# LogicTronixInc/Event-Camera-Clustering-and-Optical-Flow-Estimation

Measured on AMD Instinct MI355X. Metric: Mevents/s (downsample+cluster+corner), higher is better.
Workload: dtype u16xy/i64t (int), fp32 k-means; 1 GPU; e2e hash-downsample(8192-event windows) -> k-means k=16 (10 iters) on reps -> SAE+FAST arc corners (16384-event slices) -> 15x15 NMS; 346x260 sensor; 20004864 events/GPU/step (BASELINE configs C2-C4); events_per_gpu=20004864, events_total=20004864, preset=c4, reps_per_gpu=7697279, width=346, height=260, k=16, kmeans_iters=10, parallelism=time-window shards x1, launch=eager launches, streams=two streams sharing all CUs

## Files before the change

### event-camera-clustering-and-optical-flow-estimation_amd/csrc/corner_flags.hip

```cpp
#include "corner_common.hpp"
#include "flag_decode.hpp"

namespace {

#ifndef ECC_FLAG_THREADS
#define ECC_FLAG_THREADS 256
#endif
constexpr int kFlagThreads = ECC_FLAG_THREADS;
#ifndef ECC_FLAG_QUADS
#define ECC_FLAG_QUADS 8
#endif
constexpr int kFlagQuads = ECC_FLAG_QUADS;
constexpr int kFlagBatch = kFlagQuads * kFlagThreads;

#ifndef ECC_FLAG_GROUP
#define ECC_FLAG_GROUP 4
#endif
constexpr int kFlagGroup = ECC_FLAG_GROUP;
static_assert(kFlagQuads % kFlagGroup == 0, "a batch is whole read groups");
static_assert(kFlagTile == (uint32_t)kTile && kFlagSegWords == (uint32_t)kSegWords, "flag_decode.hpp's tile");

template <bool kStaged>
__device__ __forceinline__ uint32_t seg_word(uint32_t w, const uint32_t *sb, const uint32_t *__restrict__ rg) {
    return kStaged ? sb[w] : rg[w];
}

template <bool kStaged>
__device__ __forceinline__ uint32_t corner_bit(uint32_t v, const CornerGeom &g, uint32_t last_word, const uint32_t *sb,
                                               const uint32_t *__restrict__ rg) {
    const uint32_t x = (uint32_t)ecc::xy_x(v), y = (uint32_t)ecc::xy_y(v);
    const FlagSlot sl = flag_slot(x, y, (uint32_t)g.tiles_x, last_word);
    return (seg_word<kStaged>(sl.word, sb, rg) >> sl.bit) & flag_on_sensor(x, y, (uint32_t)g.W, (uint32_t)g.H);
}

__device__ __forceinline__ uint32_t first_bytes(int r) {
    const int rc = min(max(r, 0), 4);
    return rc >= 4 ? 0x01010101u : (0x01010101u & ((1u << (8 * (rc & 3))) - 1u));
}

template <bool kStaged, bool kCand>
__global__ void __launch_bounds__(kFlagThreads)
flags_event_kernel(const uint32_t *__restrict__ xy, CornerGeom g, const uint32_t *__restrict__ res,
                   const int32_t *__restrict__ first_border, uint8_t *__restrict__ flags, uint32_t *__restrict__ cand,
                   int32_t *__restrict__ n_cand) {
    extern __shared__ uint32_t sb[];
    __shared__ int ctot[kFlagQuads][kFlagThreads / 64];
    const int64_t s = blockIdx.x;
    const int64_t lo = s * g.S;
    const int len = (int)((lo + g.S < g.n ? lo + g.S : g.n) - lo);
    const uint32_t last_word = (uint32_t)(g.n_tiles * kSegWords - 1);
    const int live_end = s < g.first_detect ? 0 : (g.border_mode == 1 ? min(len, max(first_border[s], 0)) : len);
    const uint32_t *rg = res + s * g.seg_stride;
    const bool vec = ((lo + (int64_t)(reinterpret_cast<uintptr_t>(flags) & 3)) & 3) == 0;
    const int n4 = vec ? len / 4 : 0;
    const int lane = threadIdx.x & 63, wave = threadIdx.x >> 6;
    const __amdgpu_buffer_rsrc_t vq = ecc::buffer_view(xy + lo, (uint32_t)n4 * 16u);
    uint4 pre[kFlagQuads];
    auto load_batch = [&](int q0) {
#pragma unroll
        for (int u = 0; u < kFlagQuads; ++u)
            pre[u] = ecc::buffer_load_u128(vq, threadIdx.x * 16u, (uint32_t)(q0 + u * kFlagThreads) * 16u);
        __builtin_amdgcn_sched_barrier(0);
    };
    load_batch(0);
    if (kStaged && live_end > 0) {
        const int total = g.n_tiles * kSegWords;
        const __amdgpu_buffer_rsrc_t vr = ecc::buffer_view(rg, (uint32_t)total * 4u);
        for (int k0 = 0; k0 < total; k0 += 16 * kFlagThreads) {
            uint4 a[4];
#pragma unroll
            for (int b = 0; b < 4; ++b) a[b] = ecc::buffer_load_u128(vr, (uint32_t)(k0 + 4 * (b * kFlagThreads + (int)threadIdx.x)) * 4u);
            __builtin_amdgcn_sched_barrier(0);
#pragma unroll
            for (int b = 0; b < 4; ++b) {
                const int k = k0 + 4 * (b * kFlagThreads + (int)threadIdx.x);
                if (k + 3 < total) {
                    *reinterpret_cast<uint4 *>(sb + k) = a[b];
                } else {
                    if (k < total) sb[k] = a[b].x;
                    if (k + 1 < total) sb[k + 1] = a[b].y;
                    if (k + 2 < total) sb[k + 2] = a[b].z;
                }
            }
        }
    }
    __syncthreads();
    const int live_q = min(live_end, 4 * n4);
    const __amdgpu_buffer_rsrc_t vf = ecc::buffer_view(flags + lo, (uint32_t)n4 * 4u);
    const uint64_t lt = lane == 0 ? 0ull : (~0ull >> (64 - lane));
    int base = 0;
    uint32_t *dst = cand + lo;
    for (int q0 = 0; q0 < n4; q0 += kFlagBatch) {
        if (q0 > 0) load_batch(q0);
        uint32_t f[kFlagQuads];
        int pfx[kFlagQuads];
#pragma unroll
        for (int u0 = 0; u0 < kFlagQuads; u0 += kFlagGroup) {
            uint32_t wd[kFlagGroup][4], sh[kFlagGroup], ok[kFlagGroup];
#pragma unroll
            for (int u = 0; u < kFlagGroup; ++u) {
                const uint32_t ev[4] = {pre[u0 + u].x, pre[u0 + u].y, pre[u0 + u].z, pre[u0 + u].w};
                sh[u] = ok[u] = 0u;
#pragma unroll
                for (int k = 0; k < 4; ++k) {
                    const uint32_t x = (uint32_t)ecc::xy_x(ev[k]), y = (uint32_t)ecc::xy_y(ev[k]);
                    const FlagSlot sl = flag_slot(x, y, (uint32_t)g.tiles_x, last_word);
                    wd[u][k] = seg_word<kStaged>(sl.word, sb, rg);
                    sh[u] |= sl.bit << (8 * k);
                    ok[u] |= flag_on_sensor(x, y, (uint32_t)g.W, (uint32_t)g.H) << (8 * k);
                }
            }
#pragma unroll
            for (int u = 0; u < kFlagGroup; ++u) {
                const int i = 4 * (q0 + (u0 + u) * kFlagThreads + (int)threadIdx.x);
                uint32_t bits = 0u;
#pragma unroll
                for (int k = 0; k < 4; ++k) bits |= ((wd[u][k] >> ((sh[u] >> (8 * k)) & 31u)) & 1u) << (8 * k);
                f[u0 + u] = bits & ok[u] & first_bytes(live_q - i);
                ecc::buffer_store_u32(f[u0 + u], vf, threadIdx.x * 4u, (uint32_t)(q0 + (u0 + u) * kFlagThreads) * 4u);
            }
        }
#pragma unroll
        for (int u = 0; u < kFlagQuads; ++u) {
            if constexpr (kCand) {
                const int c = __popc(f[u]);
                const uint64_t b0 = __ballot(c & 1), b1 = __ballot(c & 2), b2 = __ballot(c & 4);
                pfx[u] = __popcll(b0 & lt) + 2 * __popcll(b1 & lt) + 4 * __popcll(b2 & lt);
                if (lane == 0) ctot[u][wave] = __popcll(b0) + 2 * __popcll(b1) + 4 * __popcll(b2);
            }
        }
        if constexpr (kCand) {
            __syncthreads();
#pragma unroll
            for (int u = 0; u < kFlagQuads; ++u) {
                int off = base + pfx[u];
#pragma unroll
                for (int w = 0; w < kFlagThreads / 64; ++w) {
                    const int tw = ctot[u][w];
                    off += w < wave ? tw : 0;
                    base += tw;
                }
                if (f[u]) {
                    if (f[u] & 0x1u) dst[off++] = pre[u].x;
                    if (f[u] & 0x100u) dst[off++] = pre[u].y;
                    if (f[u] & 0x10000u) dst[off++] = pre[u].z;
                    if (f[u] & 0x1000000u) dst[off++] = pre[u].w;
                }
            }
            __syncthreads();
        }
    }
    if constexpr (kCand) {
        if (threadIdx.x == 0) {
            for (int i = 4 * n4; i < len; ++i) {
                const uint32_t v = xy[lo + i];
                const uint32_t fb = corner_bit<kStaged>(v, g, last_word, sb, rg) & (i < live_end ? 1u : 0u);
                flags[lo + i] = (uint8_t)fb;
                if (fb) dst[base++] = v;
            }
            n_cand[s] = base;
        }
    } else {
        for (int i = 4 * n4 + threadIdx.x; i < len; i += kFlagThreads)
            flags[lo + i] = (uint8_t)(corner_bit<kStaged>(xy[lo + i], g, last_word, sb, rg) & (i < live_end ? 1u : 0u));
    }
}

}

int ecc::corner::launch_flags(ecc_ctx *ctx, hipStream_t s, const uint32_t *xy, const CornerGeom &g, const GroupImages &gi,
                              const int32_t *first_border, uint8_t *corner_flags, uint32_t *cand, int32_t *n_cand) {
    ECC_TIMED(ctx, s, "flags_kernel");
    constexpr size_t kLdsMax = kFlagDynLdsMax;
    const size_t lds = (size_t)g.n_tiles * kSegWords * sizeof(uint32_t);
    if (lds <= kLdsMax) {
        const auto fn = cand ? &flags_event_kernel<true, true> : &flags_event_kernel<true, false>;
        if (lds > 65536)
            if (int rc = ecc::allow_dynamic_lds(ctx, fn, (int)kLdsMax, "flags LDS")) return rc;
        if (cand)
            hipLaunchKernelGGL((flags_event_kernel<true, true>), dim3((unsigned)g.n_slices), dim3(kFlagThreads), lds, s,
                               xy, g, (const uint32_t *)gi.res, first_border, corner_flags, cand, n_cand);
        else
            hipLaunchKernelGGL((flags_event_kernel<true, false>), dim3((unsigned)g.n_slices), dim3(kFlagThreads), lds,
                               s, xy, g, (const uint32_t *)gi.res, first_border, corner_flags, nullptr, nullptr);
    } else {
        if (cand) return ECC_ERR_INVALID;
        hipLaunchKernelGGL((flags_event_kernel<false, false>), dim3((unsigned)g.n_slices), dim3(kFlagThreads), 0, s,
                           xy, g, (const uint32_t *)gi.res, first_border, corner_flags, nullptr, nullptr);
    }
    return ECC_OK;
}
```

Measured before the change: 44250 Mevents/s.

## Re-raster staged corner flags into sensor-order LDS bitmap, pipeline loads, pack scan

```diff
diff --git a/event-camera-clustering-and-optical-flow-estimation_amd/csrc/corner_flags.hip b/event-camera-clustering-and-optical-flow-estimation_amd/csrc/corner_flags.hip
--- a/event-camera-clustering-and-optical-flow-estimation_amd/csrc/corner_flags.hip
+++ b/event-camera-clustering-and-optical-flow-estimation_amd/csrc/corner_flags.hip
@@ -1,5 +1,6 @@
 #include "corner_common.hpp"
 #include "flag_decode.hpp"
+#include "flag_raster.hpp"
 
 namespace {
 
@@ -11,13 +12,36 @@
 #define ECC_FLAG_QUADS 8
 #endif
 constexpr int kFlagQuads = ECC_FLAG_QUADS;
-constexpr int kFlagBatch = kFlagQuads * kFlagThreads;
 
 #ifndef ECC_FLAG_GROUP
 #define ECC_FLAG_GROUP 4
 #endif
 constexpr int kFlagGroup = ECC_FLAG_GROUP;
 static_assert(kFlagQuads % kFlagGroup == 0, "a batch is whole read groups");
+#ifndef ECC_FLAG_RASTER
+#define ECC_FLAG_RASTER 1
+#endif
+constexpr bool kFlagRaster = ECC_FLAG_RASTER != 0;
+#ifndef ECC_FLAG_SCAN
+#define ECC_FLAG_SCAN 1
+#endif
+constexpr bool kFlagScan = ECC_FLAG_SCAN != 0;
+#ifndef ECC_FLAG_PIPE
+#define ECC_FLAG_PIPE 1
+#endif
+constexpr bool kFlagPipe = ECC_FLAG_PIPE != 0;
+static_assert(kFlagQuads % 2 == 0, "the quad counts are packed in pairs");
+constexpr int kFlagWaves = kFlagThreads / 64;
+constexpr int kFlagTotWords = kFlagScan ? 2 * kFlagWaves * (kFlagQuads / 2) : kFlagQuads * kFlagWaves;
+static_assert(kFlagTotWords * 4 + 4 <= 160 * 1024 - (int)kFlagDynLdsMax, "the static LDS kFlagDynLdsMax leaves room for");
+
+constexpr uint32_t kFlagListExtra = 384;
+__host__ __device__ inline uint32_t flag_lds_words(uint32_t n_tiles) {
+    const uint32_t seg = n_tiles * (uint32_t)kSegWords;
+    if (!kFlagRaster) return seg;
+    const uint32_t most = (uint32_t)(kFlagDynLdsMax / 4), want = ((seg + 3u) & ~3u) + kFlagListExtra;
+    return want < most ? want : most;
+}
 static_assert(kFlagTile == (uint32_t)kTile && kFlagSegWords == (uint32_t)kSegWords, "flag_decode.hpp's tile");
 
 template <bool kStaged>
@@ -25,12 +49,35 @@
     return kStaged ? sb[w] : rg[w];
 }
 
+template <bool kRaster>
+__device__ __forceinline__ FlagSlot flag_look(uint32_t x, uint32_t y, const CornerGeom &g, uint32_t last) {
+    if constexpr (kRaster) {
+        const uint32_t idx = flag_raster_index(x, y, (uint32_t)g.W, last);
+        return FlagSlot{idx >> 5, idx & 31u};
+    } else {
+        return flag_slot(x, y, (uint32_t)g.tiles_x, last);
+    }
+}
+
 template <bool kStaged>
-__device__ __forceinline__ uint32_t corner_bit(uint32_t v, const CornerGeom &g, uint32_t last_word, const uint32_t *sb,
+__device__ __forceinline__ uint32_t corner_bit(uint32_t v, const CornerGeom &g, uint32_t last, const uint32_t *sb,
                                                const uint32_t *__restrict__ rg) {
     const uint32_t x = (uint32_t)ecc::xy_x(v), y = (uint32_t)ecc::xy_y(v);
-    const FlagSlot sl = flag_slot(x, y, (uint32_t)g.tiles_x, last_word);
+    const FlagSlot sl = flag_look<kStaged && kFlagRaster>(x, y, g, last);
     return (seg_word<kStaged>(sl.word, sb, rg) >> sl.bit) & flag_on_sensor(x, y, (uint32_t)g.W, (uint32_t)g.H);
+}
+
+__device__ __forceinline__ void raster_or_word(uint32_t *sb, uint32_t i, uint32_t w, const CornerGeom &g) {
+    const FlagStageWord sw = flag_stage_word(i, (uint32_t)g.tiles_x, g.tx_mul, g.tx_sh);
+    while (w) {
+        const uint32_t b = (uint32_t)__builtin_ctz(w);
+        w &= w - 1u;
+        const FlagStagePixel px = flag_stage_pixel(sw, b, (uint32_t)g.W, (uint32_t)g.H);
+        if (px.set) {
+            const uint32_t idx = __umul24(px.y, (uint32_t)g.W) + px.x;
+            atomicOr(sb + (idx >> 5), 1u << (idx & 31u));
+        }
+    }
 }
 
 __device__ __forceinline__ uint32_t first_bytes(int r) {
@@ -43,45 +90,107 @@
 flags_event_kernel(const uint32_t *__restrict__ xy, CornerGeom g, const uint32_t *__restrict__ res,
                    const int32_t *__restrict__ first_border, uint8_t *__restrict__ flags, uint32_t *__restrict__ cand,
                    int32_t *__restrict__ n_cand) {
+    constexpr bool kRaster = kStaged && kFlagRaster;
     extern __shared__ uint32_t sb[];
-    __shared__ int ctot[kFlagQuads][kFlagThreads / 64];
+    __shared__ uint32_t ctot[kFlagTotWords];
+    __shared__ uint32_t n_list;
     const int64_t s = blockIdx.x;
     const int64_t lo = s * g.S;
     const int len = (int)((lo + g.S < g.n ? lo + g.S : g.n) - lo);
-    const uint32_t last_word = (uint32_t)(g.n_tiles * kSegWords - 1);
+    const uint32_t last = kRaster ? (uint32_t)(g.W * g.H - 1) : (uint32_t)(g.n_tiles * kSegWords - 1);
     const int live_end = s < g.first_detect ? 0 : (g.border_mode == 1 ? min(len, max(first_border[s], 0)) : len);
     const uint32_t *rg = res + s * g.seg_stride;
     const bool vec = ((lo + (int64_t)(reinterpret_cast<uintptr_t>(flags) & 3)) & 3) == 0;
     const int n4 = vec ? len / 4 : 0;
     const int lane = threadIdx.x & 63, wave = threadIdx.x >> 6;
     const __amdgpu_buffer_rsrc_t vq = ecc::buffer_view(xy + lo, (uint32_t)n4 * 16u);
-    uint4 pre[kFlagQuads];
-    auto load_batch = [&](int q0) {
-#pragma unroll
-        for (int u = 0; u < kFlagQuads; ++u)
-            pre[u] = ecc::buffer_load_u128(vq, threadIdx.x * 16u, (uint32_t)(q0 + u * kFlagThreads) * 16u);
+    constexpr bool kPipe = kStaged && kFlagPipe;
+    constexpr int kQ = kPipe ? kFlagQuads / 2 : kFlagQuads;
+    constexpr int kBatch = kQ * kFlagThreads;
+    static_assert(kQ % kFlagGroup == 0 && kQ % 2 == 0, "a batch is whole read groups and whole pairs");
+    uint4 pre[kQ], nxt[kPipe ? kQ : 1];
+    auto load_batch = [&](uint4(&to)[kQ], int q0) {
+#pragma unroll
+        for (int u = 0; u < kQ; ++u)
+            to[u] = ecc::buffer_load_u128(vq, threadIdx.x * 16u, (uint32_t)(q0 + u * kFlagThreads) * 16u);
         __builtin_amdgcn_sched_barrier(0);
     };
-    load_batch(0);
+    if constexpr (kPipe)
+        load_batch(reinterpret_cast<uint4(&)[kQ]>(nxt), 0);
+    else
+        load_batch(pre, 0);
     if (kStaged && live_end > 0) {
         const int total = g.n_tiles * kSegWords;
         const __amdgpu_buffer_rsrc_t vr = ecc::buffer_view(rg, (uint32_t)total * 4u);
+        const uint32_t ras4 = (flag_raster_words((uint32_t)g.W, (uint32_t)g.H) + 3u) & ~3u;
+        const uint32_t cap = kRaster ? (flag_lds_words((uint32_t)g.n_tiles) - ras4) * 4u / 6u : 0u;
+        uint32_t *const list_w = sb + ras4;
+        uint16_t *const list_i = reinterpret_cast<uint16_t *>(list_w + cap);
+        if constexpr (kRaster) {
+            for (uint32_t k = 4u * threadIdx.x; k < ras4; k += 4u * kFlagThreads)
+                *reinterpret_cast<uint4 *>(sb + k) = make_uint4(0u, 0u, 0u, 0u);
+            if (threadIdx.x == 0) n_list = 0u;
+            __syncthreads();
+        }
         for (int k0 = 0; k0 < total; k0 += 16 * kFlagThreads) {
             uint4 a[4];
 #pragma unroll
             for (int b = 0; b < 4; ++b) a[b] = ecc::buffer_load_u128(vr, (uint32_t)(k0 + 4 * (b * kFlagThreads + (int)threadIdx.x)) * 4u);
             __builtin_amdgcn_sched_barrier(0);
-#pragma unroll
-            for (int b = 0; b < 4; ++b) {
-                const int k = k0 + 4 * (b * kFlagThreads + (int)threadIdx.x);
-                if (k + 3 < total) {
-                    *reinterpret_cast<uint4 *>(sb + k) = a[b];
-                } else {
-                    if (k < total) sb[k] = a[b].x;
-                    if (k + 1 < total) sb[k + 1] = a[b].y;
-                    if (k + 2 < total) sb[k + 2] = a[b].z;
-                }
-            }
+            if constexpr (kRaster) {
+                uint32_t nz = 0u;
+#pragma unroll
+                for (int b = 0; b < 4; ++b)
+                    nz += (a[b].x != 0u) + (a[b].y != 0u) + (a[b].z != 0u) + (a[b].w != 0u);
+                const uint32_t incl = (uint32_t)ecc::wave_incl_scan((int)nz);
+                uint32_t first = 0u;
+                if (lane == 63 && incl) first = atomicAdd(&n_list, incl);
+                const uint32_t pos0 = (uint32_t)ecc::lane_value((int)first, 63) + incl - nz;
+                uint32_t pos = pos0;
+#pragma unroll
+                for (int b = 0; b < 4; ++b) {
+                    const uint32_t k = (uint32_t)(k0 + 4 * (b * kFlagThreads + (int)threadIdx.x));
+                    const uint32_t wv[4] = {a[b].x, a[b].y, a[b].z, a[b].w};
+#pragma unroll
+                    for (uint32_t c = 0; c < 4; ++c)
+                        if (wv[c]) {
+                            if (pos < cap) {
+                                list_w[pos] = wv[c];
+                                list_i[pos] = (uint16_t)(k + c);
+                            }
+                            ++pos;
+                        }
+                }
+                if (pos > cap) {
+                    pos = pos0;
+#pragma unroll 1
+                    for (uint32_t e = 0; e < 16u; ++e) {
+                        const uint32_t k = (uint32_t)k0 + 4u * ((e >> 2) * kFlagThreads + threadIdx.x) + (e & 3u);
+                        const uint32_t w = k < (uint32_t)total ? rg[k] : 0u;
+                        if (w) {
+                            if (pos >= cap) raster_or_word(sb, k, w, g);
+                            ++pos;
+                        }
+                    }
+                }
+            } else {
+#pragma unroll
+                for (int b = 0; b < 4; ++b) {
+                    const int k = k0 + 4 * (b * kFlagThreads + (int)threadIdx.x);
+                    if (k + 3 < total) {
+                        *reinterpret_cast<uint4 *>(sb + k) = a[b];
+                    } else {
+                        if (k < total) sb[k] = a[b].x;
+                        if (k + 1 < total) sb[k + 1] = a[b].y;
+                        if (k + 2 < total) sb[k + 2] = a[b].z;
+                    }
+                }
+            }
+        }
+        if constexpr (kRaster) {
+            __syncthreads();
+            const uint32_t nl = n_list < cap ? n_list : cap;
+            for (uint32_t e = threadIdx.x; e < nl; e += kFlagThreads) raster_or_word(sb, list_i[e], list_w[e], g);
         }
     }
     __syncthreads();
@@ -90,21 +199,21 @@
     const uint64_t lt = lane == 0 ? 0ull : (~0ull >> (64 - lane));
     int base = 0;
     uint32_t *dst = cand + lo;
-    for (int q0 = 0; q0 < n4; q0 += kFlagBatch) {
-        if (q0 > 0) load_batch(q0);
-        uint32_t f[kFlagQuads];
-        int pfx[kFlagQuads];
-#pragma unroll
-        for (int u0 = 0; u0 < kFlagQuads; u0 += kFlagGroup) {
+    auto run_batch = [&](int q0) {
+        const uint4(&pq)[kQ] = pre;
+        uint32_t f[kQ];
+        int pfx[kQ];
+#pragma unroll
+        for (int u0 = 0; u0 < kQ; u0 += kFlagGroup) {
             uint32_t wd[kFlagGroup][4], sh[kFlagGroup], ok[kFlagGroup];
 #pragma unroll
             for (int u = 0; u < kFlagGroup; ++u) {
-                const uint32_t ev[4] = {pre[u0 + u].x, pre[u0 + u].y, pre[u0 + u].z, pre[u0 + u].w};
+                const uint32_t ev[4] = {pq[u0 + u].x, pq[u0 + u].y, pq[u0 + u].z, pq[u0 + u].w};
                 sh[u] = ok[u] = 0u;
 #pragma unroll
                 for (int k = 0; k < 4; ++k) {
                     const uint32_t x = (uint32_t)ecc::xy_x(ev[k]), y = (uint32_t)ecc::xy_y(ev[k]);
-                    const FlagSlot sl = flag_slot(x, y, (uint32_t)g.tiles_x, last_word);
+                    const FlagSlot sl = flag_look<kRaster>(x, y, g, last);
                     wd[u][k] = seg_word<kStaged>(sl.word, sb, rg);
                     sh[u] |= sl.bit << (8 * k);
                     ok[u] |= flag_on_sensor(x, y, (uint32_t)g.W, (uint32_t)g.H) << (8 * k);
@@ -120,41 +229,83 @@
                 ecc::buffer_store_u32(f[u0 + u], vf, threadIdx.x * 4u, (uint32_t)(q0 + (u0 + u) * kFlagThreads) * 4u);
             }
         }
-#pragma unroll
-        for (int u = 0; u < kFlagQuads; ++u) {
-            if constexpr (kCand) {
+        auto write_quad = [&](int u, int off) {
+            if (f[u]) {
+                if (f[u] & 0x1u) dst[off++] = pq[u].x;
+                if (f[u] & 0x100u) dst[off++] = pq[u].y;
+                if (f[u] & 0x10000u) dst[off++] = pq[u].z;
+                if (f[u] & 0x1000000u) dst[off++] = pq[u].w;
+            }
+        };
+        if constexpr (kCand && kFlagScan) {
+            static_assert(4 * kFlagThreads < 65536, "a quad slot's flags fit a 16-bit field");
+            constexpr int kPairs = kQ / 2;
+            uint32_t *const tot = ctot + (((q0 / kBatch) & 1) ? kFlagWaves * kPairs : 0);
+            uint32_t cw[kPairs], sc[kPairs];
+#pragma unroll
+            for (int j = 0; j < kPairs; ++j) {
+                cw[j] = (uint32_t)__popc(f[2 * j]) | ((uint32_t)__popc(f[2 * j + 1]) << 16);
+                sc[j] = (uint32_t)ecc::wave_incl_scan((int)cw[j]);
+            }
+            if (lane == 63) {
+#pragma unroll
+                for (int j = 0; j < kPairs; ++j) tot[wave * kPairs + j] = sc[j];
+            }
+            __syncthreads();
+#pragma unroll
+            for (int j = 0; j < kPairs; ++j) {
+                uint32_t below = 0u, all = 0u;
+#pragma unroll
+                for (int w = 0; w < kFlagWaves; ++w) {
+                    const uint32_t tw = tot[w * kPairs + j];
+                    below += w < wave ? tw : 0u;
+                    all += tw;
+                }
+                const uint32_t ex = sc[j] - cw[j] + below;
+                write_quad(2 * j, base + (int)(ex & 0xffffu));
+                base += (int)(all & 0xffffu);
+                write_quad(2 * j + 1, base + (int)(ex >> 16));
+                base += (int)(all >> 16);
+            }
+        } else if constexpr (kCand) {
+#pragma unroll
+            for (int u = 0; u < kQ; ++u) {
                 const int c = __popc(f[u]);
                 const uint64_t b0 = __ballot(c & 1), b1 = __ballot(c & 2), b2 = __ballot(c & 4);
                 pfx[u] = __popcll(b0 & lt) + 2 * __popcll(b1 & lt) + 4 * __popcll(b2 & lt);
-                if (lane == 0) ctot[u][wave] = __popcll(b0) + 2 * __popcll(b1) + 4 * __popcll(b2);
-            }
-        }
-        if constexpr (kCand) {
-            __syncthreads();
-#pragma unroll
-            for (int u = 0; u < kFlagQuads; ++u) {
+                if (lane == 0) ctot[u * kFlagWaves + wave] = (uint32_t)(__popcll(b0) + 2 * __popcll(b1) + 4 * __popcll(b2));
+            }
+            __syncthreads();
+#pragma unroll
+            for (int u = 0; u < kQ; ++u) {
                 int off = base + pfx[u];
 #pragma unroll
-                for (int w = 0; w < kFlagThreads / 64; ++w) {
-                    const int tw = ctot[u][w];
+                for (int w = 0; w < kFlagWaves; ++w) {
+                    const int tw = (int)ctot[u * kFlagWaves + w];
                     off += w < wave ? tw : 0;
                     base += tw;
                 }
-                if (f[u]) {
-                    if (f[u] & 0x1u) dst[off++] = pre[u].x;
-                    if (f[u] & 0x100u) dst[off++] = pre[u].y;
-                    if (f[u] & 0x10000u) dst[off++] = pre[u].z;
-                    if (f[u] & 0x1000000u) dst[off++] = pre[u].w;
-                }
-            }
-            __syncthreads();
-        }
+                write_quad(u, off);
+            }
+            __syncthreads();
+        }
+    };
+    for (int q0 = 0; q0 < n4; q0 += kBatch) {
+        if constexpr (kPipe) {
+#pragma unroll
+            for (int u = 0; u < kQ; ++u) pre[u] = nxt[u];
+            __builtin_amdgcn_sched_barrier(0);
+            load_batch(reinterpret_cast<uint4(&)[kQ]>(nxt), q0 + kBatch);
+        } else {
+            if (q0 > 0) load_batch(pre, q0);
+        }
+        run_batch(q0);
     }
     if constexpr (kCand) {
         if (threadIdx.x == 0) {
             for (int i = 4 * n4; i < len; ++i) {
                 const uint32_t v = xy[lo + i];
-                const uint32_t fb = corner_bit<kStaged>(v, g, last_word, sb, rg) & (i < live_end ? 1u : 0u);
+                const uint32_t fb = corner_bit<kStaged>(v, g, last, sb, rg) & (i < live_end ? 1u : 0u);
                 flags[lo + i] = (uint8_t)fb;
                 if (fb) dst[base++] = v;
             }
@@ -162,7 +313,7 @@
         }
     } else {
         for (int i = 4 * n4 + threadIdx.x; i < len; i += kFlagThreads)
-            flags[lo + i] = (uint8_t)(corner_bit<kStaged>(xy[lo + i], g, last_word, sb, rg) & (i < live_end ? 1u : 0u));
+            flags[lo + i] = (uint8_t)(corner_bit<kStaged>(xy[lo + i], g, last, sb, rg) & (i < live_end ? 1u : 0u));
     }
 }
 
@@ -172,8 +323,9 @@
                               const int32_t *first_border, uint8_t *corner_flags, uint32_t *cand, int32_t *n_cand) {
     ECC_TIMED(ctx, s, "flags_kernel");
     constexpr size_t kLdsMax = kFlagDynLdsMax;
-    const size_t lds = (size_t)g.n_tiles * kSegWords * sizeof(uint32_t);
-    if (lds <= kLdsMax) {
+    const bool staged = (size_t)g.n_tiles * kSegWords * sizeof(uint32_t) <= kLdsMax;
+    const size_t lds = (size_t)flag_lds_words((uint32_t)g.n_tiles) * sizeof(uint32_t);
+    if (staged) {
         const auto fn = cand ? &flags_event_kernel<true, true> : &flags_event_kernel<true, false>;
         if (lds > 65536)
             if (int rc = ecc::allow_dynamic_lds(ctx, fn, (int)kLdsMax, "flags LDS")) return rc;
diff --git a/event-camera-clustering-and-optical-flow-estimation_amd/csrc/flag_raster.hpp b/event-camera-clustering-and-optical-flow-estimation_amd/csrc/flag_raster.hpp
--- /dev/null
+++ b/event-camera-clustering-and-optical-flow-estimation_amd/csrc/flag_raster.hpp
@@ -0,0 +1,31 @@
+#pragma once
+#include <cstdint>
+
+#include "flag_decode.hpp"
+
+ECC_DECODE_HD uint32_t flag_raster_words(uint32_t W, uint32_t H) { return (W * H + 31u) >> 5; }
+
+ECC_DECODE_HD uint32_t flag_raster_index(uint32_t x, uint32_t y, uint32_t W, uint32_t last_bit) {
+    const uint32_t i = ECC_UMUL24(y, W) + x;
+    return i < last_bit ? i : last_bit;
+}
+
+struct FlagStageWord {
+    uint32_t x0, y0;
+    uint32_t lp0;
+};
+ECC_DECODE_HD FlagStageWord flag_stage_word(uint32_t i, uint32_t tiles_x, uint32_t tx_mul, uint32_t tx_sh) {
+    const uint32_t tile = i / kFlagSegWords;
+    const uint32_t ty = magic_quot(tile, tx_mul, tx_sh), tx = tile - ty * tiles_x;
+    return FlagStageWord{tx * kFlagTile, ty * kFlagTile, 32u * (i - tile * kFlagSegWords)};
+}
+
+struct FlagStagePixel {
+    uint32_t x, y, set;
+};
+ECC_DECODE_HD FlagStagePixel flag_stage_pixel(const FlagStageWord &sw, uint32_t b, uint32_t W, uint32_t H) {
+    const uint32_t lp = sw.lp0 + b;
+    const uint32_t ly = ECC_UMUL24(lp, 4682u) >> 16;
+    const uint32_t x = sw.x0 + (lp - ly * kFlagTile), y = sw.y0 + ly;
+    return FlagStagePixel{x, y, (lp < kFlagTile * kFlagTile && x < W && y < H) ? 1u : 0u};
+}
```

Measured after the change: 45070 Mevents/s, median of 6. 1.9% higher.
